# lmmontoya-ai/taboo-brittleness

Measured on AMD Instinct MI355X. Metric: prompts/sec SAE-ablation sweep Gemma-2-9B @L32, higher is better.
Workload: dtype bf16

## Files before the change

### taboo_brittleness_amd/csrc/api.h

```cpp
#pragma once
#include <hip/hip_runtime.h>
#include <stdint.h>

void tb_rmsnorm(const uint16_t* x, const uint16_t* w, uint16_t* y, int M, int D, float eps, hipStream_t st);
void tb_add_rmsnorm2(uint16_t* h, const uint16_t* o, const uint16_t* w_post, const uint16_t* w_next, uint16_t* x,
                     int M, int D, float eps, hipStream_t st);
void tb_embed_rmsnorm(const int32_t* ids, const uint16_t* E, const uint16_t* w, uint16_t* h, uint16_t* x, int M,
                      int D, int V, float scale, float eps, hipStream_t st);
void tb_rope_qkv_cache(const uint16_t* qkv, const int32_t* pos, const int32_t* slot_of_row, const float* cos_t,
                       const float* sin_t, uint16_t* q_out, uint16_t* kc, uint16_t* vc, int M, int Hq, int Hkv,
                       int HD, int S, int max_pos, hipStream_t st);
void tb_rope_qkv_cache_part(const float* part, int ks, const int32_t* pos, const int32_t* slot_of_row,
                            const float* cos_t, const float* sin_t, uint16_t* q_out, uint16_t* kc, uint16_t* vc, int M,
                            int Hq, int Hkv, int HD, int S, int max_pos, hipStream_t st);
void tb_kv_fanout(uint16_t* kc, uint16_t* vc, const int32_t* src_row, const int32_t* slot, const int32_t* pos, int M,
                  int nlayers, int slots, int Hkv, int S, int HD, hipStream_t st);
int tb_attention_lds_bytes(int HD);
int tb_attention_split_rows(int n, bool prefix);
void tb_attention(const uint16_t* q, const uint16_t* kc, const uint16_t* vc, uint16_t* out, const int32_t* pos,
                  const int32_t* slot, int B, int T, int Hq, int Hkv, int HD, int S, float scale, float softcap,
                  int window, hipStream_t st, const uint16_t* pkc = nullptr, const uint16_t* pvc = nullptr,
                  const int32_t* pslot = nullptr, const int32_t* plen = nullptr);
void tb_attention_varlen(const uint16_t* q, const uint16_t* kc, const uint16_t* vc, uint16_t* out, const int32_t* pos,
                         const int32_t* blk, int nblk, int Hq, int Hkv, int HD, int S, float scale, float softcap,
                         int window, hipStream_t st, int bw = 3, const uint16_t* pkc = nullptr,
                         const uint16_t* pvc = nullptr);
void tb_geglu(const uint16_t* gu, uint16_t* out, int M, int F, hipStream_t st);
void tb_argmax_rows(const uint16_t* logits, int32_t* out, int R, int V, float cap, hipStream_t st);
void tb_row_lse(const uint16_t* logits, float* lse, int R, int V, float cap, int emulate_bf16, hipStream_t st);
void tb_gather_probs(const uint16_t* logits, const float* lse, const int32_t* ids, float* out, int R, int K, int V,
                     int round_bf16, const int32_t* rowmap, hipStream_t st);
void tb_lens_colsum(const uint16_t* logits, const float* lse, const uint8_t* mask, const int32_t* excl, float* acc,
                    int B, int T, int V, int accumulate, int round_bf16, const int32_t* offs, float* cum,
                    const int32_t* rowmap, hipStream_t st);
int tb_topk_chunks(int R, int V);
void tb_topk_rows(const float* x, float* vals, int32_t* idx, int R, int V, int K, float* wv, int32_t* wi, int C,
                  hipStream_t st);
void tb_xent_rows(const uint16_t* logits, const int32_t* tgt, float* nll, int R, int V, float cap, int emulate_bf16,
                  hipStream_t st);
void tb_register_softcap_table(float cap, const uint16_t* tab);
void tb_decode_head(const uint16_t* logits, const int32_t* tgt, int32_t* nxt, float* nll_self, float* nll_tgt, int R,
                    int V, float cap, hipStream_t st);
bool tb_decode_head_stats(const uint16_t* logits, const int32_t* tgt, int off, float* stats, int R, int V, float cap,
                          hipStream_t st);
int tb_decode_head_track(const uint16_t* logits, const int32_t* tgt, int32_t* nxt, float* nll_self, float* nll_tgt,
                         const int32_t* track, int T, int n_rank, float* logp, int32_t* rank, const int64_t* col, int W,
                         int R, int V, float cap, hipStream_t st);
int tb_head_shift(const uint16_t* logits, const uint16_t* base, const int32_t* rowmap, float* kl, float* kl_rev, int R,
                  int Rb, int V, float cap, hipStream_t st);
void tb_head_merge(const float* part, int npart, const int32_t* tgt, const float* tgt_logit, int32_t* nxt,
                   float* nll_self, float* nll_tgt, float* lse, int M, int V, hipStream_t st);
void tb_head_fused4(const uint16_t* A, const uint16_t* W, float* part, float cap, const int32_t* tgt,
                    float* tgt_logit, int32_t* nxt, float* nll_self, float* nll_tgt, int M, int N, int K, hipStream_t st);
void tb_gemm4_qkv_rope(const uint16_t* A, const uint16_t* W, const int32_t* pos, const int32_t* slot_of_row,
                       const uint16_t* cs, uint16_t* q_out, uint16_t* kc, uint16_t* vc, int M, int K,
                       int Hq, int Hkv, int S, int max_pos, int tile_rows, hipStream_t st, const uint16_t* a2 = nullptr,
                       int k0 = 0);
bool tb_register_softcap_compact(float cap, const uint16_t* tab, int lo, int hi, float sat);
bool tb_softcap_compact(const uint16_t* x, float* y, int n, float cap, hipStream_t st);
bool tb_gemm4_ok(int M, int N, int K);
int tb_gemm4_set_pipe(int on);
int tb_gemm4_splitk_ks(int M, int N, int K, int tile_rows);
int tb_gemm4_splitk_part(const uint16_t* A, const uint16_t* W, float* ws, int M, int N, int K, int tile_rows, int ks,
                         hipStream_t st);
void tb_add_rmsnorm2_part(uint16_t* h, const float* part, int ks, const uint16_t* w_post, const uint16_t* w_next,
                          uint16_t* x, int M, int D, float eps, hipStream_t st);
void tb_gemm4_splitk(const uint16_t* A, const uint16_t* W, uint16_t* out, float* ws, int M, int N, int K, int ldo,
                     int epi, int tile_rows, int ks, hipStream_t st);
void tb_row_combine(const int64_t* ptr, const float* coef, float* out, int B, int T, int V, hipStream_t st);
bool tb_random_basis_ok(int D);
void tb_random_basis(const uint64_t* seeds, const int32_t* ranks, const int64_t* rows, int n, int D, float* table,
                     hipStream_t st, int qu = 1);
void tb_gemm4(const uint16_t* A, const uint16_t* W, void* C, const float* bias, const float* thr, int M, int N, int K,
              int ldc, int epi, int tile_rows, hipStream_t st, const uint16_t* a2 = nullptr, int k0 = 0);
void tb_gemm_nt(const uint16_t* A, const uint16_t* W, void* C, const float* bias, const float* thr, int M, int N,
                int K, int ldc, int epi, hipStream_t st);
void tb_lowrank_edit(uint16_t* h, uint16_t* x_next, const uint8_t* apply, const int32_t* idx, const int32_t* cnt,
                     int mmax, const void* E, const void* Dm, int table_f32, const float* bias, const float* thr,
                     const float* pre_bias, float alpha, const uint16_t* w_next, float eps, int M, int D,
                     float* coef_out, hipStream_t st, const float* val = nullptr);
void tb_interchange_edit(uint16_t* h, uint16_t* x_next, const uint8_t* apply, const int32_t* idx, const int32_t* cnt,
                         int mmax, const void* E, const void* Dm, int table_f32, const float* bias, const float* thr,
                         const float* pre_bias, float alpha, const uint16_t* w_next, float eps, int M, int D,
                         float* coef_out, const uint16_t* donor, const int32_t* src, int n_donor, float* dcoef_out,
                         hipStream_t st);
void tb_matched_noise_edit(uint16_t* h, uint16_t* x_next, const uint8_t* apply, const int32_t* idx,
                           const int32_t* cnt, int mmax, const void* E, const void* Dm, int table_f32,
                           const float* bias, const float* thr, const float* pre_bias, float alpha,
                           const uint16_t* w_next, float eps, int M, int D, float* coef_out, const float* val,
                           const uint64_t* seeds, const int32_t* pos, float* norm_out, hipStream_t st);
void tb_sae_splice_edit(uint16_t* h, uint16_t* x_next, const uint8_t* apply, const int32_t* src_row,
                        const float* acts, int n_act_rows, int L, const int32_t* idx, const int32_t* cnt, int mmax,
                        const void* Wdec, int table_f32, const float* b_dec, float alpha, const uint16_t* w_next,
                        float eps, int M, int D, hipStream_t st);
void tb_flag_compact(const uint8_t* flags, int n, int32_t* rows, int cap, int32_t* inv, hipStream_t st);
void tb_sae_decode_sparse(const float* acts, const void* Wdec, int table_f32, const float* b_dec, uint16_t* out_bf16,
                          float* out_f32, int M, int L, int D, hipStream_t st);
void tb_latent_score(const float* acts, const float* p, const uint8_t* spike, const int32_t* seg, float* out,
                     float* spike_mean, float* corr, int G, int L, hipStream_t st);
void tb_latent_effect(const float* acts, const uint16_t* X, const float* V, int v_per_row, const void* Wdec,
                      int table_f32, const int32_t* seg, float* score, float* eff, int R, int G, int L, int D,
// ... 56 lines not shown
```

### taboo_brittleness_amd/csrc/attention.hip

```cpp
#include <stdlib.h>

#include "common.h"
#include "api.h"

int tb_attention_lds_bytes(int HD) {
  const int VSTR = HD + 16, PSTR = 40;
  const int stage = 4 * 32 * VSTR * 2 + 4 * 16 * PSTR * 2;
  return ((stage + 128 * 4 + 15) / 16) * 16;
}

namespace {

typedef short v4i16 __attribute__((ext_vector_type(4)));

__device__ __forceinline__ v4i16 ds_read_tr16(const uint16_t* lds_ptr) {
  return __builtin_amdgcn_ds_read_tr16_b64_v4i16((__attribute__((address_space(3))) v4i16*)(lds_ptr));
}

__device__ __forceinline__ bf16x8 as_bf16x8(const uint4& u) { return __builtin_bit_cast(bf16x8, u); }

template <int HD, int G>
__global__ void __launch_bounds__(256) attn_cache_kernel(
    const uint16_t* __restrict__ q, const uint16_t* __restrict__ kc, const uint16_t* __restrict__ vc,
    uint16_t* __restrict__ out, const int32_t* __restrict__ pos, const int32_t* __restrict__ slot, int T, int Hq,
// ... 450 lines not shown
  if constexpr (KDB == 2) {
    uint4 ka[KS], kb[KS];
    kload(t0, ka);
    for (int t = t0; t <= t1; t += 2) {
      if (t + 1 <= t1) kload(t + 1, kb);
      score(t, ka);
      if (t + 1 <= t1) {
        if (t + 2 <= t1) kload(t + 2, ka);
        score(t + 1, kb);
      }
    }
  } else {
    for (int t = t0; t <= t1; ++t) {
      uint4 ka[KS];
      kload(t, ka);
      score(t, ka);
    }
  }
  __builtin_amdgcn_fence(__ATOMIC_RELEASE, "wavefront");
  __builtin_amdgcn_wave_barrier();
  __builtin_amdgcn_fence(__ATOMIC_ACQUIRE, "wavefront");
  float inv_l[G];
#pragma unroll
  for (int h = 0; h < G; ++h) {
    float* sh = sc + h * SS;
    float m = -INFINITY;
    for (int j = kmin + lane; j <= kmax; j += 64) m = fmaxf(m, sh[j]);
    m = wave_max(m);
    float l = 0.f;
    for (int j = kmin + lane; j <= kmax; j += 64) {
      const float pw = m > -INFINITY ? rbf(__expf(sh[j] - m)) : 0.f;
      sh[j] = pw;
      l += pw;
    }
    l = wave_sum(l);
    inv_l[h] = l > 0.f ? 1.f / l : 0.f;
  }
  __builtin_amdgcn_fence(__ATOMIC_RELEASE, "wavefront");
  __builtin_amdgcn_wave_barrier();
  __builtin_amdgcn_fence(__ATOMIC_ACQUIRE, "wavefront");
  float o[G][DPL];
#pragma unroll
  for (int h = 0; h < G; ++h)
#pragma unroll
    for (int d = 0; d < DPL; ++d) o[h][d] = 0.f;
  auto accum = [&](int j, const VT (&v)[VCH]) {
#pragma unroll
    for (int u = 0; u < VCH; ++u) {
      if (j + u > kmax) break;
      float vf[DPL];
      vrow_t<DPL>::unpack(v[u], vf);
#pragma unroll
      for (int h = 0; h < G; ++h) {
        const float pw = sc[h * SS + j + u];
#pragma unroll
        for (int d = 0; d < DPL; ++d) o[h][d] += pw * vf[d];
      }
    }
  };
  for (int j = kmin; j <= kmax; j += 2 * VCH) {
    if (j + VCH <= kmax) vload(j + VCH, vb);
    accum(j, va);
    if (j + VCH <= kmax) {
      if (j + 2 * VCH <= kmax) vload(j + 2 * VCH, va);
      accum(j + VCH, vb);
    }
  }
#pragma unroll
  for (int h = 0; h < G; ++h) {
    float r[DPL];
#pragma unroll
    for (int d = 0; d < DPL; ++d) r[d] = o[h][d] * inv_l[h];
    uint16_t* dst = ob + h * HD + lane * DPL;
    if constexpr (DPL == 4) {
      *reinterpret_cast<uint2*>(dst) = make_uint2(pack2(r[0], r[1]), pack2(r[2], r[3]));
    } else {
      *reinterpret_cast<uint32_t*>(dst) = pack2(r[0], r[1]);
    }
  }
}


template <int HD, int G>
__global__ void __launch_bounds__(256) attn_tail_exact_kernel(
    const uint16_t* __restrict__ q, const uint16_t* __restrict__ kc, const uint16_t* __restrict__ vc,
    uint16_t* __restrict__ out, const int32_t* __restrict__ pos, int Hq, int Hkv, int S, float scale, float softcap,
    int window, const int32_t* __restrict__ blk, int nitems, int bw, const uint16_t* __restrict__ pkc,
    const uint16_t* __restrict__ pvc) {
  constexpr int P = 16 / G;
  constexpr int KS = HD / 32;
  constexpr int DPL = HD / 64;
  constexpr int VCH = 8;
  using VT = typename vrow_t<DPL>::type;
  extern __shared__ __attribute__((aligned(16))) char smem[];
  const int lane = threadIdx.x & 63, wid = threadIdx.x >> 6;
  const int item = blockIdx.x * 4 + wid;
  if (item >= nitems) return;
  const int SS = (S + 15) & ~15;
  float* sc = reinterpret_cast<float*>(smem) + (size_t)wid * 16 * SS;
  const int bi = item / Hkv, kh = item % Hkv;
  const int rbase = blk[bw * bi], nvalid = blk[bw * bi + 1], cs = blk[bw * bi + 2];
  const int ps = bw == 5 ? blk[bw * bi + 3] : 0, np = bw == 5 ? blk[bw * bi + 4] : 0;
  const int grp = lane >> 4, col = lane & 15;
  const uint16_t* kbase = kc + ((size_t)cs * Hkv + kh) * (size_t)S * HD;
  const uint16_t* vbase = vc + ((size_t)cs * Hkv + kh) * (size_t)S * HD;
  const uint16_t* kpre = kbase;
  const uint16_t* vpre = vbase;
  if (np > 0) {
    kpre = pkc + ((size_t)ps * Hkv + kh) * (size_t)S * HD;
    vpre = pvc + ((size_t)ps * Hkv + kh) * (size_t)S * HD;
  }
  auto rpos = [&](int r) -> int { return (r / G) < nvalid ? pos[(size_t)rbase + r / G] : -1; };
  auto rkmax = [&](int p) -> int { return p < S ? p : S - 1; };
  auto rkmin = [&](int p) -> int {
    int k = 0;
    if (window > 0) { k = p - window + 1; if (k < 0) k = 0; }
    return k;
  };
  int kmaxb = -1, kminb = 1 << 30;
#pragma unroll
  for (int r = 0; r < 16; ++r) {
    const int p = rpos(r);
    if (p >= 0) { kmaxb = max(kmaxb, rkmax(p)); kminb = min(kminb, rkmin(p)); }
  }
  uint16_t* orow0 = out + (size_t)rbase * Hq * HD;
  if (kmaxb < 0) {
    for (int e = lane; e < nvalid * G * HD; e += 64) {
      const int t = e / (G * HD), rem = e % (G * HD);
      orow0[(size_t)t * Hq * HD + kh * G * HD + rem] = 0;
    }
    return;
  }
  const int pA = rpos(col);
  bf16x8 qa[KS];
  {
    const uint16_t* qrow = q + (((size_t)rbase + col / G) * Hq + kh * G + col % G) * HD + grp * 8;
#pragma unroll
    for (int ks = 0; ks < KS; ++ks) {
      uint4 u = {0, 0, 0, 0};
      if (pA >= 0) u = *reinterpret_cast<const uint4*>(qrow + ks * 32);
      qa[ks] = as_bf16x8(u);
    }
  }
  int pC[4];
#pragma unroll
  for (int i = 0; i < 4; ++i) pC[i] = rpos(4 * grp + i);
  const float inv_cap = softcap > 0.f ? 1.f / softcap : 0.f;
  for (int t = kminb >> 4; t <= kmaxb >> 4; ++t) {
    const int kk = t * 16 + col;
    const int kr = kk < kminb ? kminb : (kk > kmaxb ? kmaxb : kk);
    const uint16_t* krow = (kr < np ? kpre : kbase) + (size_t)kr * HD + grp * 8;
    f32x4 acc = {0.f, 0.f, 0.f, 0.f};
#pragma unroll
    for (int ks = 0; ks < KS; ++ks)
      acc = __builtin_amdgcn_mfma_f32_16x16x32_bf16(qa[ks], as_bf16x8(*reinterpret_cast<const uint4*>(krow + ks * 32)),
                                                    acc, 0, 0, 0);
    float sv[4];
#pragma unroll
    for (int i = 0; i < 4; ++i) {
      float s = acc[i] * scale;
      if (softcap > 0.f) s = tanhf(s * inv_cap) * softcap;
      const int p = pC[i];
      sv[i] = (p >= 0 && kk >= rkmin(p) && kk <= rkmax(p)) ? s : -INFINITY;
    }
    if (kk < SS) *reinterpret_cast<float4*>(sc + (size_t)kk * 16 + 4 * grp) = make_float4(sv[0], sv[1], sv[2], sv[3]);
  }
  __builtin_amdgcn_fence(__ATOMIC_RELEASE, "wavefront");
// ... 1 lines not shown
  __builtin_amdgcn_fence(__ATOMIC_ACQUIRE, "wavefront");
  float inv_l[16];
#pragma unroll
  for (int r = 0; r < 16; ++r) {
    const int p = rpos(r);
    inv_l[r] = 0.f;
    if (p < 0) {
      for (int j = kminb + lane; j <= kmaxb; j += 64) sc[(size_t)j * 16 + r] = 0.f;
      continue;
    }
    const int k0 = rkmin(p), k1 = rkmax(p);
    float m = -INFINITY;
    for (int j = k0 + lane; j <= k1; j += 64) m = fmaxf(m, sc[(size_t)j * 16 + r]);
    m = wave_max(m);
    float l = 0.f;
    for (int j = k0 + lane; j <= k1; j += 64) {
      const float pw = m > -INFINITY ? rbf(__expf(sc[(size_t)j * 16 + r] - m)) : 0.f;
      sc[(size_t)j * 16 + r] = pw;
      l += pw;
    }
    l = wave_sum(l);
    inv_l[r] = l > 0.f ? 1.f / l : 0.f;
    for (int j = kminb + lane; j <= kmaxb; j += 64)
      if (j < k0 || j > k1) sc[(size_t)j * 16 + r] = 0.f;
  }
  __builtin_amdgcn_fence(__ATOMIC_RELEASE, "wavefront");
  __builtin_amdgcn_wave_barrier();
  __builtin_amdgcn_fence(__ATOMIC_ACQUIRE, "wavefront");
  float o[16][DPL];
#pragma unroll
  for (int r = 0; r < 16; ++r)
#pragma unroll
    for (int d = 0; d < DPL; ++d) o[r][d] = 0.f;
  auto vload = [&](int j, VT (&v)[VCH]) {
#pragma unroll
    for (int u = 0; u < VCH; ++u) {
      const int jj = j + u <= kmaxb ? j + u : kmaxb;
      v[u] = *reinterpret_cast<const VT*>((jj < np ? vpre : vbase) + (size_t)jj * HD + lane * DPL);
    }
  };
  auto accum = [&](int j, const VT (&v)[VCH]) {
#pragma unroll
    for (int u = 0; u < VCH; ++u) {
      if (j + u > kmaxb) break;
      float vf[DPL];
      vrow_t<DPL>::unpack(v[u], vf);
      const float4* pr = reinterpret_cast<const float4*>(sc + (size_t)(j + u) * 16);
#pragma unroll
      for (int r4 = 0; r4 < 4; ++r4) {
        const float4 pw4 = pr[r4];
        const float pwv[4] = {pw4.x, pw4.y, pw4.z, pw4.w};
#pragma unroll
        for (int i = 0; i < 4; ++i)
#pragma unroll
          for (int d = 0; d < DPL; ++d) o[4 * r4 + i][d] += pwv[i] * vf[d];
      }
    }
  };
  VT va[VCH], vb[VCH];
  vload(kminb, va);
  for (int j = kminb; j <= kmaxb; j += 2 * VCH) {
    if (j + VCH <= kmaxb) vload(j + VCH, vb);
    accum(j, va);
    if (j + VCH <= kmaxb) {
      if (j + 2 * VCH <= kmaxb) vload(j + 2 * VCH, va);
      accum(j + VCH, vb);
    }
  }
#pragma unroll
  for (int r = 0; r < 16; ++r) {
    if (r / G >= nvalid) continue;
    float v[DPL];
#pragma unroll
    for (int d = 0; d < DPL; ++d) v[d] = o[r][d] * inv_l[r];
    uint16_t* dst = out + (((size_t)rbase + r / G) * Hq + kh * G + r % G) * HD + lane * DPL;
    if constexpr (DPL == 4) {
      *reinterpret_cast<uint2*>(dst) = make_uint2(pack2(v[0], v[1]), pack2(v[2], v[3]));
    } else {
      *reinterpret_cast<uint32_t*>(dst) = pack2(v[0], v[1]);
    }
  }
}


template <int HD, int G>
__global__ void __launch_bounds__(256) attn_decode_split_kernel(
    const uint16_t* __restrict__ q, const uint16_t* __restrict__ kc, const uint16_t* __restrict__ vc,
    uint16_t* __restrict__ out, const int32_t* __restrict__ pos, const int32_t* __restrict__ slot, int Hq, int Hkv,
    int S, float scale, float softcap, int window, const uint16_t* __restrict__ pkc, const uint16_t* __restrict__ pvc,
    const int32_t* __restrict__ pslot, const int32_t* __restrict__ plen) {
  constexpr int KS = HD / 32;
  constexpr int PARTS = 4 / G;
  constexpr int DPW = HD / PARTS / 64;
  constexpr int VCH = 8;
  static_assert(PARTS * G == 4 && (DPW == 2 || DPW == 4), "geometry");
  using VT = typename vrow_t<DPW>::type;
  extern __shared__ __attribute__((aligned(16))) char smem[];
  const int b = blockIdx.x, kh = blockIdx.y;
  const int lane = threadIdx.x & 63, w = threadIdx.x >> 6;
  const int grp = lane >> 4, col = lane & 15;
  const int SS = (S + 15) & ~15;
  float* sc = reinterpret_cast<float*>(smem);
  uint16_t* ql = reinterpret_cast<uint16_t*>(sc + (size_t)G * SS);
  uint16_t* ob = out + ((size_t)b * Hq + kh * G) * HD;
  const int p = pos[b];
  if (p < 0) {
    for (int e = threadIdx.x; e < G * HD; e += 256) ob[e] = 0;
    return;
  }
  const int kmax = p < S ? p : S - 1;
  int kmin = 0;
  if (window > 0) { kmin = p - window + 1; if (kmin < 0) kmin = 0; }
  const int cs = slot[b];
  const uint16_t* kbase = kc + ((size_t)cs * Hkv + kh) * (size_t)S * HD;
  const uint16_t* vbase = vc + ((size_t)cs * Hkv + kh) * (size_t)S * HD;
  int np = 0;
  const uint16_t* kpre = kbase;
  const uint16_t* vpre = vbase;
  if (plen != nullptr) {
    np = plen[b];
    if (np > 0) {
      const size_t po = ((size_t)pslot[b] * Hkv + kh) * (size_t)S * HD;
      kpre = pkc + po;
      vpre = pvc + po;
    }
  }
  const int h = w / PARTS, d0 = (w % PARTS) * (HD / PARTS) + lane * DPW;
  auto vload = [&](int j, VT (&v)[VCH]) {
#pragma unroll
    for (int u = 0; u < VCH; ++u) {
      const int jj = j + u <= kmax ? j + u : kmax;
      v[u] = *reinterpret_cast<const VT*>((jj < np ? vpre : vbase) + (size_t)jj * HD + d0);
    }
  };
  VT va[VCH], vb[VCH];
  vload(kmin, va);
  {
    const uint16_t* qrow = q + ((size_t)b * Hq + kh * G) * HD;
    for (int e = threadIdx.x; e < G * HD / 8; e += 256)
      *reinterpret_cast<uint4*>(ql + e * 8) = *reinterpret_cast<const uint4*>(qrow + e * 8);
  }
  __syncthreads();
  const float inv_cap = softcap > 0.f ? 1.f / softcap : 0.f;
  const uint16_t* qlr = ql + (col % G) * HD + grp * 8;
  const int t0 = kmin >> 4, t1 = kmax >> 4;
  for (int t = t0 + w; t <= t1; t += 4) {
    uint4 kf[KS];
    const int kk = t * 16 + col;
    const int kr = kk < kmin ? kmin : (kk > kmax ? kmax : kk);
    const uint16_t* krow = (kr < np ? kpre : kbase) + (size_t)kr * HD + grp * 8;
#pragma unroll
    for (int ks = 0; ks < KS; ++ks) kf[ks] = *reinterpret_cast<const uint4*>(krow + ks * 32);
    f32x4 acc = {0.f, 0.f, 0.f, 0.f};
#pragma unroll
    for (int ks = 0; ks < KS; ++ks)
      acc = __builtin_amdgcn_mfma_f32_16x16x32_bf16(as_bf16x8(*reinterpret_cast<const uint4*>(qlr + ks * 32)),
                                                    as_bf16x8(kf[ks]), acc, 0, 0, 0);
    if (grp == 0) {
#pragma unroll
      for (int hh = 0; hh < G; ++hh) {
        float s = acc[hh] * scale;
        if (softcap > 0.f) s = tanhf(s * inv_cap) * softcap;
        sc[hh * SS + kk] = (kk >= kmin && kk <= kmax) ? s : -INFINITY;
      }
    }
  }
  __syncthreads();
  float m[G];
#pragma unroll
  for (int hh = 0; hh < G; ++hh) {
    const float* sh = sc + hh * SS;
    float mm = -INFINITY;
    for (int j = kmin + lane; j <= kmax; j += 64) mm = fmaxf(mm, sh[j]);
    m[hh] = wave_max(mm);
  }
  __syncthreads();
#pragma unroll
  for (int hh = 0; hh < G; ++hh) {
    float* sh = sc + hh * SS;
    for (int j = kmin + lane + 64 * w; j <= kmax; j += 256)
      sh[j] = m[hh] > -INFINITY ? rbf(__expf(sh[j] - m[hh])) : 0.f;
  }
  __syncthreads();
  float inv_l;
  {
    const float* sh = sc + h * SS;
    float l = 0.f;
    for (int j = kmin + lane; j <= kmax; j += 64) l += sh[j];
    l = wave_sum(l);
    inv_l = l > 0.f ? 1.f / l : 0.f;
  }
  float o[DPW];
#pragma unroll
  for (int d = 0; d < DPW; ++d) o[d] = 0.f;
  const float* ph = sc + h * SS;
  auto accum = [&](int j, const VT (&v)[VCH]) {
#pragma unroll
    for (int u = 0; u < VCH; ++u) {
      if (j + u > kmax) break;
      float vf[DPW];
      vrow_t<DPW>::unpack(v[u], vf);
      const float pw = ph[j + u];
#pragma unroll
      for (int d = 0; d < DPW; ++d) o[d] += pw * vf[d];
    }
  };
  for (int j = kmin; j <= kmax; j += 2 * VCH) {
    if (j + VCH <= kmax) vload(j + VCH, vb);
    accum(j, va);
    if (j + VCH <= kmax) {
      if (j + 2 * VCH <= kmax) vload(j + 2 * VCH, va);
      accum(j + VCH, vb);
    }
  }
  float r[DPW];
#pragma unroll
  for (int d = 0; d < DPW; ++d) r[d] = o[d] * inv_l;
  uint16_t* dst = ob + h * HD + d0;
  if constexpr (DPW == 4) {
    *reinterpret_cast<uint2*>(dst) = make_uint2(pack2(r[0], r[1]), pack2(r[2], r[3]));
  } else {
    *reinterpret_cast<uint32_t*>(dst) = pack2(r[0], r[1]);
  }
}

template <int HD, int G>
void launch_attn(const uint16_t* q, const uint16_t* kc, const uint16_t* vc, uint16_t* out, const int32_t* pos,
                 const int32_t* slot, int B, int T, int Hq, int Hkv, int S, float scale, float softcap, int window,
                 hipStream_t st, const int32_t* blk = nullptr, int nblk = 0, int bw = 3,
                 const uint16_t* pkc = nullptr, const uint16_t* pvc = nullptr) {
  constexpr int P = 16 / G;
  const size_t lds = (size_t)tb_attention_lds_bytes(HD);
  static bool attr_set = false;
  if (!attr_set) {
    (void)hipFuncSetAttribute(reinterpret_cast<const void*>(&attn_cache_kernel<HD, G>),
                              hipFuncAttributeMaxDynamicSharedMemorySize, (int)lds);
    attr_set = true;
  }
  if (blk != nullptr && S <= 512) {
    const size_t lds_t = (size_t)4 * 16 * ((S + 15) & ~15) * sizeof(float);
    static size_t attr_tail = 65536;
    if (lds_t > attr_tail) {
      (void)hipFuncSetAttribute(reinterpret_cast<const void*>(&attn_tail_exact_kernel<HD, G>),
                                hipFuncAttributeMaxDynamicSharedMemorySize, 160 * 1024);
      attr_tail = 160 * 1024;
    }
    const int nitems = nblk * Hkv;
    hipLaunchKernelGGL((attn_tail_exact_kernel<HD, G>), dim3((nitems + 3) / 4), dim3(256), lds_t, st, q, kc, vc, out,
                       pos, Hq, Hkv, S, scale, softcap, window, blk, nitems, bw, pkc, pvc);
    return;
  }
  if (blk != nullptr) {
    dim3 grid(nblk, Hkv, 1);
    hipLaunchKernelGGL((attn_cache_kernel<HD, G>), grid, dim3(256), lds, st, q, kc, vc, out, pos, slot, T, Hq, Hkv,
                       S, scale, softcap, window, blk, bw, pkc, pvc);
    return;
  }
  dim3 grid((T + P - 1) / P, Hkv, B);
  hipLaunchKernelGGL((attn_cache_kernel<HD, G>), grid, dim3(256), lds, st, q, kc, vc, out, pos, slot, T, Hq, Hkv, S,
                     scale, softcap, window, (const int32_t*)nullptr);
}


int g_attn_split_rows[2] = {64, 64};

template <int HD, int G>
void launch_attn_decode(const uint16_t* q, const uint16_t* kc, const uint16_t* vc, uint16_t* out, const int32_t* pos,
                        const int32_t* slot, int B, int Hq, int Hkv, int S, float scale, float softcap, int window,
                        const uint16_t* pkc, const uint16_t* pvc, const int32_t* pslot, const int32_t* plen,
                        hipStream_t st) {
  if constexpr (HD == 256 && (G == 2 || G == 4)) {
    if (S <= 2048 && B <= g_attn_split_rows[pkc != nullptr ? 1 : 0]) {
      const size_t lds_s = (size_t)G * ((S + 15) & ~15) * sizeof(float) + (size_t)G * HD * 2;
      hipLaunchKernelGGL((attn_decode_split_kernel<HD, G>), dim3(B, Hkv), dim3(256), lds_s, st, q, kc, vc, out, pos,
                         slot, Hq, Hkv, S, scale, softcap, window, pkc, pvc, pslot, plen);
      return;
    }
  }
  if (S <= 2048) {
    int nwh = Hkv % 4 == 0 ? 4 : (Hkv % 2 == 0 ? 2 : 1);
    auto wave_lds = [&](int n) { return (size_t)n * G * ((S + 15) & ~15) * sizeof(float) + (size_t)n * G * HD * 2; };
    while (nwh > 1 && wave_lds(nwh) > 160 * 1024) nwh >>= 1;
    const size_t lds_w = wave_lds(nwh);
    static size_t wave_attr = 65536;
    if (lds_w > wave_attr) {
      (void)hipFuncSetAttribute(reinterpret_cast<const void*>(&attn_decode_wave_kernel<HD, G>),
                                hipFuncAttributeMaxDynamicSharedMemorySize, 160 * 1024);
      wave_attr = 160 * 1024;
    }
    hipLaunchKernelGGL((attn_decode_wave_kernel<HD, G>), dim3(B, Hkv / nwh), dim3(64 * nwh), lds_w, st, q, kc, vc, out,
                       pos, slot, Hq, Hkv, S, scale, softcap, window, pkc, pvc, pslot, plen);
    return;
  }
  const size_t lds = ((size_t)G * ((S + 15) & ~15) + 4 * G * HD + 3 * G + 2) * sizeof(float);
  static size_t attr_set = 0;
  if (lds > attr_set && lds > 65536) {
    (void)hipFuncSetAttribute(reinterpret_cast<const void*>(&attn_decode_kernel<HD, G>),
                              hipFuncAttributeMaxDynamicSharedMemorySize, (int)lds);
    attr_set = lds;
  }
  hipLaunchKernelGGL((attn_decode_kernel<HD, G>), dim3(B, Hkv), dim3(256), lds, st, q, kc, vc, out, pos, slot, Hq,
                     Hkv, S, scale, softcap, window, pkc, pvc, pslot, plen);
}

}

int tb_attention_split_rows(int n, bool prefix) {
  const int old = g_attn_split_rows[prefix ? 1 : 0];
  if (n >= 0) g_attn_split_rows[prefix ? 1 : 0] = n;
  return old;
}

void tb_attention(const uint16_t* q, const uint16_t* kc, const uint16_t* vc, uint16_t* out, const int32_t* pos,
                  const int32_t* slot, int B, int T, int Hq, int Hkv, int HD, int S, float scale, float softcap,
                  int window, hipStream_t st, const uint16_t* pkc, const uint16_t* pvc, const int32_t* pslot,
                  const int32_t* plen) {
  if (B <= 0 || T <= 0) return;
  const int G = Hq / Hkv;
  if (T == 1 && S <= 8192) {
#define TB_DEC_CASE(hd, g)                                                                                   \
  if (HD == hd && G == g) {                                                                                  \
    launch_attn_decode<hd, g>(q, kc, vc, out, pos, slot, B, Hq, Hkv, S, scale, softcap, window, pkc, pvc,    \
                              pslot, plen, st);                                                              \
    return;                                                                                                  \
  }
    TB_DEC_CASE(256, 2)
    TB_DEC_CASE(256, 1)
    TB_DEC_CASE(256, 4)
    TB_DEC_CASE(128, 2)
    TB_DEC_CASE(128, 1)
    TB_DEC_CASE(128, 4)
#undef TB_DEC_CASE
  }
#define TB_ATTN_CASE(hd, g)                                                                                   \
  if (HD == hd && G == g) {                                                                                  \
    launch_attn<hd, g>(q, kc, vc, out, pos, slot, B, T, Hq, Hkv, S, scale, softcap, window, st);             \
    return;                                                                                                  \
  }
  TB_ATTN_CASE(256, 2)
  TB_ATTN_CASE(256, 1)
  TB_ATTN_CASE(256, 4)
  TB_ATTN_CASE(128, 2)
  TB_ATTN_CASE(128, 1)
  TB_ATTN_CASE(128, 4)
#undef TB_ATTN_CASE
}

void tb_attention_varlen(const uint16_t* q, const uint16_t* kc, const uint16_t* vc, uint16_t* out, const int32_t* pos,
                         const int32_t* blk, int nblk, int Hq, int Hkv, int HD, int S, float scale, float softcap,
                         int window, hipStream_t st, int bw, const uint16_t* pkc, const uint16_t* pvc) {
  if (nblk <= 0) return;
  const int G = Hq / Hkv;
#define TB_VL_CASE(hd, g)                                                                                    \
  if (HD == hd && G == g) {                                                                                  \
    launch_attn<hd, g>(q, kc, vc, out, pos, nullptr, 0, 0, Hq, Hkv, S, scale, softcap, window, st, blk, nblk,  \
                       bw, pkc, pvc);                                                                        \
    return;                                                                                                  \
  }
  TB_VL_CASE(256, 2)
  TB_VL_CASE(256, 1)
  TB_VL_CASE(256, 4)
  TB_VL_CASE(128, 2)
  TB_VL_CASE(128, 1)
  TB_VL_CASE(128, 4)
#undef TB_VL_CASE
}
```

### taboo_brittleness_amd/csrc/bindings.cpp

```cpp
#include <torch/extension.h>
#include <ATen/hip/impl/HIPStreamMasqueradingAsCUDA.h>
#include <c10/core/DeviceGuard.h>

#include <cstdlib>

#include "api.h"

namespace {

hipStream_t cur_stream() { return c10::hip::getCurrentHIPStreamMasqueradingAsCUDA().stream(); }

#define CHECK_DEV(t) TORCH_CHECK((t).is_cuda(), #t " must be a GPU tensor")
#define CHECK_CONTIG(t) TORCH_CHECK((t).is_contiguous(), #t " must be contiguous")
#define CHECK_BF16(t) TORCH_CHECK((t).scalar_type() == at::kBFloat16, #t " must be bfloat16")
#define CHECK_F32(t) TORCH_CHECK((t).scalar_type() == at::kFloat, #t " must be float32")
#define CHECK_I32(t) TORCH_CHECK((t).scalar_type() == at::kInt, #t " must be int32")
#define CHECK_U8(t) TORCH_CHECK((t).scalar_type() == at::kByte || (t).scalar_type() == at::kBool, #t " must be uint8/bool")
#define IN_BF16(t) CHECK_DEV(t); CHECK_CONTIG(t); CHECK_BF16(t)
#define IN_F32(t) CHECK_DEV(t); CHECK_CONTIG(t); CHECK_F32(t)
#define IN_I32(t) CHECK_DEV(t); CHECK_CONTIG(t); CHECK_I32(t)
#define IN_U8(t) CHECK_DEV(t); CHECK_CONTIG(t); CHECK_U8(t)

bool debug_checks() {
  static const bool on = [] {
// ... 1123 lines not shown
                     c10::optional<torch::Tensor> l_len_lo, int64_t nb, int64_t S) {
  IN_I64(rep); IN_I64(U); IN_I32(tok); IN_I32(pos); IN_I32(slot); IN_I32(s_tok); IN_I32(s_pos); IN_I32(s_slot);
  const int64_t B = tok.numel();
  TORCH_CHECK(nb >= 0 && nb <= B && rep.numel() >= nb && pos.numel() == B && slot.numel() == B &&
              s_tok.numel() >= nb && s_pos.numel() >= nb && s_slot.numel() >= nb && U.numel() == 1,
              "share_lo_gather shapes");
  const bool kp = kp_slot.has_value() && kp_slot->defined();
  const int32_t *ks = nullptr, *kl = nullptr;
  int32_t *ls = nullptr, *ll = nullptr;
  if (kp) {
    TORCH_CHECK(kp_len_lo.has_value() && l_slot.has_value() && l_len_lo.has_value(), "share_lo_gather: prefix set");
    IN_I32((*kp_slot)); IN_I32((*kp_len_lo)); IN_I32((*l_slot)); IN_I32((*l_len_lo));
    TORCH_CHECK(kp_slot->numel() == B && kp_len_lo->numel() == B && l_slot->numel() >= nb && l_len_lo->numel() >= nb,
                "share_lo_gather: prefix shapes");
    ks = kp_slot->data_ptr<int32_t>(); kl = kp_len_lo->data_ptr<int32_t>();
    ls = l_slot->data_ptr<int32_t>(); ll = l_len_lo->data_ptr<int32_t>();
  }
  c10::DeviceGuard g(tok.device());
  tb_share_lo_gather(rep.data_ptr<int64_t>(), U.data_ptr<int64_t>(), tok.data_ptr<int32_t>(), pos.data_ptr<int32_t>(),
                     slot.data_ptr<int32_t>(), s_tok.data_ptr<int32_t>(), s_pos.data_ptr<int32_t>(),
                     s_slot.data_ptr<int32_t>(), ks, kl, ls, ll, (int)nb, (int)B, (int)S, cur_stream());
}

void capture_rows(torch::Tensor store, torch::Tensor h, torch::Tensor pos, torch::Tensor slot, int64_t T) {
  IN_BF16(store); IN_BF16(h); IN_I32(pos); IN_I32(slot);
  TORCH_CHECK(store.dim() == 3 && h.size(-1) == store.size(2) && store.size(2) % 8 == 0, "capture_rows: shapes");
  const int64_t D = store.size(2), n = h.numel() / D;
  TORCH_CHECK(T >= 1 && n % T == 0 && pos.numel() == n && slot.numel() >= n / T, "capture_rows: rows / pos / slot");
  if (debug_checks() && n > 0) {
    const auto sl = slot.narrow(0, 0, n / T);
    TORCH_CHECK(sl.min().item<int>() >= 0 && sl.max().item<int>() < store.size(0), "capture_rows: slot out of range");
  }
  c10::DeviceGuard g(h.device());
  tb_capture_rows(bf(store), cbf(h), pos.data_ptr<int32_t>(), slot.data_ptr<int32_t>(), (int)n, (int)T,
                  (int)store.size(1), (int)D, cur_stream());
}

void row_gather(torch::Tensor src, torch::Tensor idx, torch::Tensor out) {
  IN_BF16(src); IN_BF16(out); CHECK_DEV(idx); CHECK_CONTIG(idx);
  TORCH_CHECK(idx.scalar_type() == at::kLong || idx.scalar_type() == at::kInt, "row_gather: idx int32/int64");
  const int64_t D = src.size(-1), n = idx.numel();
  TORCH_CHECK(D % 8 == 0 && out.size(-1) == D && out.numel() >= n * D, "row_gather: shapes");
  if (debug_checks() && n > 0)
    TORCH_CHECK(idx.min().item<int64_t>() >= 0 && idx.max().item<int64_t>() < src.numel() / D,
                "row_gather: index out of range");
  c10::DeviceGuard g(src.device());
  tb_row_gather(bf(out), cbf(src), idx.data_ptr(), idx.scalar_type() == at::kLong, (int)n, (int)D, cur_stream());
}

void share_group(torch::Tensor gid, torch::Tensor tok, torch::Tensor rep, torch::Tensor grp, torch::Tensor src,
                 torch::Tensor U, int64_t nb, int64_t act, bool first, int64_t V) {
  IN_I64(gid); IN_I32(tok); IN_I64(rep); IN_I64(grp); IN_I32(src); IN_I64(U);
  TORCH_CHECK(nb >= 0 && nb <= tb_share_group_max_rows() && gid.numel() >= nb && tok.numel() >= nb &&
              rep.numel() >= nb && grp.numel() >= nb && src.numel() >= nb && U.numel() == 1, "share_group shapes");
  c10::DeviceGuard g(gid.device());
  tb_share_group(gid.data_ptr<int64_t>(), tok.data_ptr<int32_t>(), rep.data_ptr<int64_t>(), grp.data_ptr<int64_t>(),
                 src.data_ptr<int32_t>(), U.data_ptr<int64_t>(), (int)nb, (int)act, first ? 1 : 0, V, cur_stream());
}
int64_t share_group_max_rows() { return tb_share_group_max_rows(); }

int64_t p2p_header_bytes() { return tb_p2p_header_bytes(); }
int64_t p2p_max_ranks() { return tb_p2p_max_ranks(); }

}

PYBIND11_MODULE(TORCH_EXTENSION_NAME, m) {
  m.doc() = "taboo_brittleness_amd gfx950 kernels";
  using namespace py::literals;
  const auto a2 = "a2"_a = py::none();
  m.def("rmsnorm", &rmsnorm);
  m.def("add_rmsnorm2", &add_rmsnorm2);
  m.def("embed_rmsnorm", &embed_rmsnorm);
  m.def("rope_qkv_cache", &rope_qkv_cache);
  m.def("rope_qkv_cache_part", &rope_qkv_cache_part);
  m.def("kv_fanout", &kv_fanout);
  m.def("decode_pre", &decode_pre);
  m.def("decode_post", &decode_post);
  m.def("share_lo_gather", &share_lo_gather);
  m.def("capture_rows", &capture_rows);
  m.def("row_gather", &row_gather);
  m.def("share_group", &share_group);
  m.def("share_group_max_rows", &share_group_max_rows);
  m.def("attention_split_rows", [](int64_t n, bool prefix) { return (int64_t)tb_attention_split_rows((int)n, prefix); });
  m.def("attention", &attention);
  m.def("attention_prefix", &attention_prefix);
  m.def("attention_varlen", &attention_varlen);
  m.def("attention_varlen_prefix", &attention_varlen_prefix);
  m.def("geglu", &geglu);
  m.def("argmax_rows", &argmax_rows);
  m.def("row_lse", &row_lse);
  m.def("gather_probs", &gather_probs);
  m.def("lens_colsum", &lens_colsum);
  m.def("topk_rows", &topk_rows);
  m.def("xent_rows", &xent_rows);
  m.def("decode_head", &decode_head);
  m.def("decode_head_stats", &decode_head_stats);
  m.def("decode_head_track", &decode_head_track);
  m.def("head_shift", &head_shift);
  m.def("register_softcap_table", &register_softcap_table);
  m.def("register_softcap_compact", &register_softcap_compact);
  m.def("softcap_compact", &softcap_compact);
  m.def("gemm_nt", &gemm_nt);
  m.def("gemm4", &gemm4, "A"_a, "W"_a, "C"_a, "bias"_a, "thr"_a, "epi"_a, "tile_rows"_a, a2);
  m.def("gemm4_ok", &gemm4_ok);
  m.def("gemm4_set_pipe", &gemm4_set_pipe);
  m.def("gemm_ring", &gemm_ring, "A"_a, "W"_a, "C"_a, "epi"_a, "bm"_a, "bn"_a, "var"_a, a2);
  m.def("gemm_ring_ok", &gemm_ring_ok);
  m.def("gemm_ring_tiles", &gemm_ring_tiles);
  m.def("gemm_ring_qkv_rope", &gemm_ring_qkv_rope, "x"_a, "w"_a, "pos"_a, "slot_of_row"_a, "cs"_a, "q_out"_a,
        "kc"_a, "vc"_a, "Hq"_a, "Hkv"_a, "bm"_a, "bn"_a, "var"_a, a2);
  m.def("gemm4_splitk", &gemm4_splitk);
  m.def("gemm4_splitk_ks", &gemm4_splitk_ks);
  m.def("gemm4_splitk_part", &gemm4_splitk_part);
  m.def("add_rmsnorm2_part", &add_rmsnorm2_part);
  m.def("gemm4_qkv_rope", &gemm4_qkv_rope, "x"_a, "w"_a, "pos"_a, "slot_of_row"_a, "cs"_a, "q_out"_a, "kc"_a,
        "vc"_a, "Hq"_a, "Hkv"_a, "tile_rows"_a, a2);
  m.def("lora_t", &lora_t);
  m.def("lora_t_chunks", &lora_t_chunks);
  m.def("row_combine", &row_combine);
  m.def("random_basis", &random_basis);
  m.def("lora_t_ok", &lora_t_ok);
  m.def("head_fused", &head_fused);
  m.def("lens_gemm", &lens_gemm);
  m.def("lowrank_edit", &lowrank_edit);
  m.def("latent_affine_edit", &latent_affine_edit);
  m.def("matched_noise_edit", &matched_noise_edit);
  m.def("interchange_edit", &interchange_edit);
  m.def("sae_decode_sparse", &sae_decode_sparse);
  m.def("sae_splice_edit", &sae_splice_edit);
  m.def("flag_compact", &flag_compact);
  m.def("latent_score", &latent_score);
  m.def("latent_effect", &latent_effect);
  m.def("lens_track", &lens_track);
  m.def("attention_lds_bytes", &attention_lds_bytes);
  m.def("p2p_alloc", &p2p_alloc);
  m.def("p2p_free", &p2p_free);
  m.def("p2p_get_handle", &p2p_get_handle);
  m.def("p2p_open_handle", &p2p_open_handle);
  m.def("p2p_close_handle", &p2p_close_handle);
  m.def("p2p_allreduce", &p2p_allreduce);
  m.def("p2p_allgather", &p2p_allgather);
  m.def("vp_head_merge", &vp_head_merge);
  m.def("slot_copy", &slot_copy);
  m.def("vp_lse_merge", &vp_lse_merge);
  m.def("vp_topk_merge", &vp_topk_merge);
  m.def("p2p_read_error", &p2p_read_error);
  m.def("p2p_header_bytes", &p2p_header_bytes);
  m.def("p2p_max_ranks", &p2p_max_ranks);
}
```

Baseline: 2670.

## Add MFMA-based exact tail attention kernel and keep VALU path selectable

```diff
diff --git a/taboo_brittleness_amd/csrc/api.h b/taboo_brittleness_amd/csrc/api.h
--- a/taboo_brittleness_amd/csrc/api.h
+++ b/taboo_brittleness_amd/csrc/api.h
@@ -17,6 +17,7 @@
                   int nlayers, int slots, int Hkv, int S, int HD, hipStream_t st);
 int tb_attention_lds_bytes(int HD);
 int tb_attention_split_rows(int n, bool prefix);
+int tb_attention_tail_mode(int n);
 void tb_attention(const uint16_t* q, const uint16_t* kc, const uint16_t* vc, uint16_t* out, const int32_t* pos,
                   const int32_t* slot, int B, int T, int Hq, int Hkv, int HD, int S, float scale, float softcap,
                   int window, hipStream_t st, const uint16_t* pkc = nullptr, const uint16_t* pvc = nullptr,
diff --git a/taboo_brittleness_amd/csrc/attention.hip b/taboo_brittleness_amd/csrc/attention.hip
--- a/taboo_brittleness_amd/csrc/attention.hip
+++ b/taboo_brittleness_amd/csrc/attention.hip
@@ -556,7 +556,7 @@
 
 
 template <int HD, int G>
-__global__ void __launch_bounds__(256) attn_tail_exact_kernel(
+__global__ void __launch_bounds__(256) attn_tail_exact_valu_kernel(
     const uint16_t* __restrict__ q, const uint16_t* __restrict__ kc, const uint16_t* __restrict__ vc,
     uint16_t* __restrict__ out, const int32_t* __restrict__ pos, int Hq, int Hkv, int S, float scale, float softcap,
     int window, const int32_t* __restrict__ blk, int nitems, int bw, const uint16_t* __restrict__ pkc,
@@ -724,6 +724,238 @@
   }
 }
 
+template <int HD, int G>
+__global__ void __launch_bounds__(256, 3) attn_tail_exact_kernel(
+    const uint16_t* __restrict__ q, const uint16_t* __restrict__ kc, const uint16_t* __restrict__ vc,
+    uint16_t* __restrict__ out, const int32_t* __restrict__ pos, int Hq, int Hkv, int S, float scale, float softcap,
+    int window, const int32_t* __restrict__ blk, int nblk, int bw, const uint16_t* __restrict__ pkc,
+    const uint16_t* __restrict__ pvc) {
+  constexpr int KS = HD / 32;
+  constexpr int DT = HD / 16;
+  constexpr int VQ = DT / 8;
+  constexpr int VGR = 2;
+  constexpr int VCH = 4 * VGR;
+  extern __shared__ __attribute__((aligned(16))) char smem[];
+  const int lane = threadIdx.x & 63;
+  const int wid = __builtin_amdgcn_readfirstlane((int)(threadIdx.x >> 6));
+  const int item = (int)blockIdx.x * 4 + wid;
+  const int bi = item / Hkv, kh = item % Hkv;
+  if (bi >= nblk) return;
+  const int SS = (S + 15) & ~15;
+  float* sc = reinterpret_cast<float*>(smem) + (size_t)wid * 16 * SS;
+  const int rbase = blk[bw * bi], nvalid = blk[bw * bi + 1], cs = blk[bw * bi + 2];
+  const int ps = bw == 5 ? blk[bw * bi + 3] : 0, np = bw == 5 ? blk[bw * bi + 4] : 0;
+  const int grp = lane >> 4, col = lane & 15;
+  const uint16_t* kbase = kc + ((size_t)cs * Hkv + kh) * (size_t)S * HD;
+  const uint16_t* vbase = vc + ((size_t)cs * Hkv + kh) * (size_t)S * HD;
+  const uint16_t* kpre = kbase;
+  const uint16_t* vpre = vbase;
+  if (np > 0) {
+    kpre = pkc + ((size_t)ps * Hkv + kh) * (size_t)S * HD;
+    vpre = pvc + ((size_t)ps * Hkv + kh) * (size_t)S * HD;
+  }
+  auto rpos = [&](int r) -> int { return (r / G) < nvalid ? pos[(size_t)rbase + r / G] : -1; };
+  auto rkmax = [&](int p) -> int { return p < S ? p : S - 1; };
+  auto rkmin = [&](int p) -> int {
+    int k = 0;
+    if (window > 0) { k = p - window + 1; if (k < 0) k = 0; }
+    return k;
+  };
+  int kmaxb = -1, kminb = 1 << 30, kmin_hi = -1;
+#pragma unroll
+  for (int r = 0; r < 16; r += G) {
+    const int p = rpos(r);
+    if (p >= 0) {
+      kmaxb = max(kmaxb, rkmax(p));
+      kminb = min(kminb, rkmin(p));
+      kmin_hi = max(kmin_hi, rkmin(p));
+    }
+  }
+  if (kmaxb < 0) {
+    uint16_t* orow0 = out + (size_t)rbase * Hq * HD;
+    for (int e = lane; e < nvalid * G * HD; e += 64) {
+      const int t = e / (G * HD), rem = e % (G * HD);
+      orow0[(size_t)t * Hq * HD + kh * G * HD + rem] = 0;
+    }
+    return;
+  }
+  const bool uniform = kmin_hi == kminb;
+  auto vload = [&](int j, uint4 (&v)[VGR][VQ]) {
+#pragma unroll
+    for (int g = 0; g < VGR; ++g) {
+      const int jj = min(j + 4 * g + grp, kmaxb);
+      const uint16_t* vr = (jj < np ? vpre : vbase) + (size_t)jj * HD + col * DT;
+#pragma unroll
+      for (int x = 0; x < VQ; ++x) v[g][x] = *reinterpret_cast<const uint4*>(vr + 8 * x);
+    }
+  };
+  uint4 va[VGR][VQ], vb[VGR][VQ];
+  vload(kminb, va);
+  const int pA = rpos(col);
+  bf16x8 qa[KS];
+  {
+    const uint16_t* qrow = q + (((size_t)rbase + col / G) * Hq + kh * G + col % G) * HD + grp * 8;
+#pragma unroll
+    for (int ks = 0; ks < KS; ++ks) {
+      uint4 u = {0, 0, 0, 0};
+      if (pA >= 0) u = *reinterpret_cast<const uint4*>(qrow + ks * 32);
+      qa[ks] = as_bf16x8(u);
+    }
+  }
+  int k0C[4], k1C[4];
+#pragma unroll
+  for (int i = 0; i < 4; ++i) {
+    const int p = rpos(4 * grp + i);
+    k0C[i] = p >= 0 ? rkmin(p) : 1;
+    k1C[i] = p >= 0 ? rkmax(p) : 0;
+  }
+  const float inv_cap = softcap > 0.f ? 1.f / softcap : 0.f;
+  auto kload = [&](int t, uint4 (&kf)[KS]) {
+    const int kk = t * 16 + col;
+    const int kr = kk < kminb ? kminb : (kk > kmaxb ? kmaxb : kk);
+    const uint16_t* krow = (kr < np ? kpre : kbase) + (size_t)kr * HD + grp * 8;
+#pragma unroll
+    for (int ks = 0; ks < KS; ++ks) kf[ks] = *reinterpret_cast<const uint4*>(krow + ks * 32);
+  };
+  auto score = [&](int t, const uint4 (&kf)[KS]) {
+    const int kk = t * 16 + col;
+    f32x4 acc = {0.f, 0.f, 0.f, 0.f};
+#pragma unroll
+    for (int ks = 0; ks < KS; ++ks)
+      acc = __builtin_amdgcn_mfma_f32_16x16x32_bf16(qa[ks], as_bf16x8(kf[ks]), acc, 0, 0, 0);
+    float sv[4];
+#pragma unroll
+    for (int i = 0; i < 4; ++i) {
+      float s = acc[i] * scale;
+      if (softcap > 0.f) s = tanhf(s * inv_cap) * softcap;
+      sv[i] = (kk >= k0C[i] && kk <= k1C[i]) ? s : -INFINITY;
+    }
+    *reinterpret_cast<float4*>(sc + (size_t)kk * 16 + 4 * grp) = make_float4(sv[0], sv[1], sv[2], sv[3]);
+  };
+  {
+    const int t0 = kminb >> 4, t1 = kmaxb >> 4;
+    uint4 ka[KS], kb[KS];
+    kload(t0, ka);
+    for (int t = t0; t <= t1; t += 2) {
+      if (t + 1 <= t1) kload(t + 1, kb);
+      score(t, ka);
+      if (t + 1 <= t1) {
+        if (t + 2 <= t1) kload(t + 2, ka);
+        score(t + 1, kb);
+      }
+    }
+  }
+  if (kminb + VCH <= kmaxb) vload(kminb + VCH, vb);
+  __builtin_amdgcn_fence(__ATOMIC_RELEASE, "wavefront");
+  __builtin_amdgcn_wave_barrier();
+  __builtin_amdgcn_fence(__ATOMIC_ACQUIRE, "wavefront");
+  auto uni = [](float v) -> float {
+    return __int_as_float(__builtin_amdgcn_readfirstlane(__float_as_int(v)));
+  };
+  float invC[4] = {0.f, 0.f, 0.f, 0.f};
+  if (uniform) {
+    float m[16], l[16];
+#pragma unroll
+    for (int r = 0; r < 16; ++r) { m[r] = -INFINITY; l[r] = 0.f; }
+    for (int j = kminb + lane; j <= kmaxb; j += 64) {
+      const float4* pr = reinterpret_cast<const float4*>(sc + (size_t)j * 16);
+#pragma unroll
+      for (int r4 = 0; r4 < 4; ++r4) {
+        const float4 s4 = pr[r4];
+        m[4 * r4] = fmaxf(m[4 * r4], s4.x); m[4 * r4 + 1] = fmaxf(m[4 * r4 + 1], s4.y);
+        m[4 * r4 + 2] = fmaxf(m[4 * r4 + 2], s4.z); m[4 * r4 + 3] = fmaxf(m[4 * r4 + 3], s4.w);
+      }
+    }
+#pragma unroll
+    for (int r = 0; r < 16; ++r) m[r] = wave_max(m[r]);
+    for (int j = kminb + lane; j <= kmaxb; j += 64) {
+      float4* pr = reinterpret_cast<float4*>(sc + (size_t)j * 16);
+#pragma unroll
+      for (int r4 = 0; r4 < 4; ++r4) {
+        const float4 s4 = pr[r4];
+        const float sv[4] = {s4.x, s4.y, s4.z, s4.w};
+        float pw[4];
+#pragma unroll
+        for (int i = 0; i < 4; ++i) {
+          const float mr = m[4 * r4 + i];
+          pw[i] = (sv[i] == -INFINITY || !(mr > -INFINITY)) ? 0.f : rbf(__expf(sv[i] - mr));
+          l[4 * r4 + i] += pw[i];
+        }
+        pr[r4] = make_float4(pw[0], pw[1], pw[2], pw[3]);
+      }
+    }
+#pragma unroll
+    for (int r = 0; r < 16; ++r) {
+      const float lt = wave_sum(l[r]);
+      const float inv = uni(lt > 0.f ? 1.f / lt : 0.f);
+      invC[r % 4] = grp == r / 4 ? inv : invC[r % 4];
+    }
+  } else {
+#pragma unroll
+    for (int r = 0; r < 16; ++r) {
+      const int p = rpos(r);
+      if (p < 0) {
+        for (int j = kminb + lane; j <= kmaxb; j += 64) sc[(size_t)j * 16 + r] = 0.f;
+        continue;
+      }
+      const int k0 = rkmin(p), k1 = rkmax(p);
+      float m = -INFINITY;
+      for (int j = k0 + lane; j <= k1; j += 64) m = fmaxf(m, sc[(size_t)j * 16 + r]);
+      m = wave_max(m);
+      float l = 0.f;
+      for (int j = k0 + lane; j <= k1; j += 64) {
+        const float pw = m > -INFINITY ? rbf(__expf(sc[(size_t)j * 16 + r] - m)) : 0.f;
+        sc[(size_t)j * 16 + r] = pw;
+        l += pw;
+      }
+      l = wave_sum(l);
+      const float inv = uni(l > 0.f ? 1.f / l : 0.f);
+      invC[r % 4] = grp == r / 4 ? inv : invC[r % 4];
+      for (int j = kminb + lane; j <= kmaxb; j += 64)
+        if (j < k0 || j > k1) sc[(size_t)j * 16 + r] = 0.f;
+    }
+  }
+  __builtin_amdgcn_fence(__ATOMIC_RELEASE, "wavefront");
+  __builtin_amdgcn_wave_barrier();
+  __builtin_amdgcn_fence(__ATOMIC_ACQUIRE, "wavefront");
+  f32x4 o[DT];
+#pragma unroll
+  for (int t = 0; t < DT; ++t) o[t] = (f32x4){0.f, 0.f, 0.f, 0.f};
+  auto accum = [&](int j, const uint4 (&v)[VGR][VQ]) {
+#pragma unroll
+    for (int g = 0; g < VGR; ++g) {
+      if (j + 4 * g > kmaxb) break;
+      const int key = j + 4 * g + grp;
+      const float pw = sc[(size_t)min(key, kmaxb) * 16 + col];
+      const float a = key <= kmaxb ? pw : 0.f;
+      float vf[DT];
+#pragma unroll
+      for (int x = 0; x < VQ; ++x) unpack8(v[g][x], vf + 8 * x);
+#pragma unroll
+      for (int t = 0; t < DT; ++t) o[t] = __builtin_amdgcn_mfma_f32_16x16x4f32(a, vf[t], o[t], 0, 0, 0);
+    }
+  };
+  for (int j = kminb; j <= kmaxb; j += 2 * VCH) {
+    accum(j, va);
+    if (j + VCH <= kmaxb) {
+      if (j + 2 * VCH <= kmaxb) vload(j + 2 * VCH, va);
+      accum(j + VCH, vb);
+      if (j + 3 * VCH <= kmaxb) vload(j + 3 * VCH, vb);
+    }
+  }
+#pragma unroll
+  for (int i = 0; i < 4; ++i) {
+    const int r = 4 * grp + i;
+    if (r / G >= nvalid) continue;
+    float v[DT];
+#pragma unroll
+    for (int t = 0; t < DT; ++t) v[t] = o[t][i] * invC[i];
+    uint16_t* dst = out + (((size_t)rbase + r / G) * Hq + kh * G + r % G) * HD + col * DT;
+#pragma unroll
+    for (int x = 0; x < VQ; ++x) *reinterpret_cast<uint4*>(dst + 8 * x) = pack8(v + 8 * x);
+  }
+}
+
 
 template <int HD, int G>
 __global__ void __launch_bounds__(256) attn_decode_split_kernel(
@@ -866,6 +1098,8 @@
   }
 }
 
+int g_attn_tail_mode = 1;
+
 template <int HD, int G>
 void launch_attn(const uint16_t* q, const uint16_t* kc, const uint16_t* vc, uint16_t* out, const int32_t* pos,
                  const int32_t* slot, int B, int T, int Hq, int Hkv, int S, float scale, float softcap, int window,
@@ -885,11 +1119,18 @@
     if (lds_t > attr_tail) {
       (void)hipFuncSetAttribute(reinterpret_cast<const void*>(&attn_tail_exact_kernel<HD, G>),
                                 hipFuncAttributeMaxDynamicSharedMemorySize, 160 * 1024);
+      (void)hipFuncSetAttribute(reinterpret_cast<const void*>(&attn_tail_exact_valu_kernel<HD, G>),
+                                hipFuncAttributeMaxDynamicSharedMemorySize, 160 * 1024);
       attr_tail = 160 * 1024;
     }
     const int nitems = nblk * Hkv;
+    if (g_attn_tail_mode == 0) {
+      hipLaunchKernelGGL((attn_tail_exact_valu_kernel<HD, G>), dim3((nitems + 3) / 4), dim3(256), lds_t, st, q, kc, vc,
+                         out, pos, Hq, Hkv, S, scale, softcap, window, blk, nitems, bw, pkc, pvc);
+      return;
+    }
     hipLaunchKernelGGL((attn_tail_exact_kernel<HD, G>), dim3((nitems + 3) / 4), dim3(256), lds_t, st, q, kc, vc, out,
-                       pos, Hq, Hkv, S, scale, softcap, window, blk, nitems, bw, pkc, pvc);
+                       pos, Hq, Hkv, S, scale, softcap, window, blk, nblk, bw, pkc, pvc);
     return;
   }
   if (blk != nullptr) {
@@ -950,6 +1191,12 @@
 int tb_attention_split_rows(int n, bool prefix) {
   const int old = g_attn_split_rows[prefix ? 1 : 0];
   if (n >= 0) g_attn_split_rows[prefix ? 1 : 0] = n;
+  return old;
+}
+
+int tb_attention_tail_mode(int n) {
+  const int old = g_attn_tail_mode;
+  if (n == 0 || n == 1) g_attn_tail_mode = n;
   return old;
 }
 
diff --git a/taboo_brittleness_amd/csrc/bindings.cpp b/taboo_brittleness_amd/csrc/bindings.cpp
--- a/taboo_brittleness_amd/csrc/bindings.cpp
+++ b/taboo_brittleness_amd/csrc/bindings.cpp
@@ -1229,6 +1229,7 @@
   m.def("share_group", &share_group);
   m.def("share_group_max_rows", &share_group_max_rows);
   m.def("attention_split_rows", [](int64_t n, bool prefix) { return (int64_t)tb_attention_split_rows((int)n, prefix); });
+  m.def("attention_tail_mode", [](int64_t n) { return (int64_t)tb_attention_tail_mode((int)n); });
   m.def("attention", &attention);
   m.def("attention_prefix", &attention_prefix);
   m.def("attention_varlen", &attention_varlen);
```

Measured after the change: 2692, median of 6. About the same (+0.9%).
